# upowai/upow

Hardware: AMD Instinct MI355X
Metric: sha256_pow_hashrate_MH/s (higher is better)
Workload: dtype uint32; 1 GPU; model=upow v2 block header PoW (108 B, single SHA-256, nibble-prefix target), global_batch=4294967296, seq_len=108, parallelism=dp1, nonces_per_rank_step=4294967296, device=gpu, kernel_variant=0

## Files before the change

csrc/bindings.cpp:

```cpp
#include <pybind11/numpy.h>
#include <pybind11/pybind11.h>
#include <pybind11/stl.h>

#include <cstring>
#include <malloc.h>
#include <stdexcept>

#include "native.h"
#include "sha256_common.h"
#include "thread_pool.h"

namespace py = pybind11;
using namespace upow;

namespace upow {
void register_txcodec(py::module_& m);
void register_ledger_writer(py::module_& m);
void register_gov_index(py::module_& m);
void register_stall_probe(py::module_& m);
void register_log_appender(py::module_& m);
void register_http_wire(py::module_& m);
void register_mempool_index(py::module_& m);
void register_jsonspan(py::module_& m);
void register_utxo_host(py::module_& m);
// ... 82 lines not shown
            if (!PyUnicode_Check(o)) throw py::type_error("transaction hex must be str");
            Py_ssize_t sz = 0;
            const char* p = PyUnicode_AsUTF8AndSize(o, &sz);
            if (!p) throw py::error_already_set();
            if (nc[k] < 0 || nc[k] > int64_t(sz)) throw py::value_error("sha256_hex_prefixes: prefix longer than the hex");
            src[size_t(k)] = p;
        }
        std::string out(size_t(n) * 32, '\0');
        {
            py::gil_scoped_release rel;
            HostPool::get().parallel_for(n, threads, [&](int64_t k) {
                host_sha256(reinterpret_cast<const uint8_t*>(src[size_t(k)]), size_t(nc[k]),
                            reinterpret_cast<uint8_t*>(&out[size_t(k) * 32]));
            });
        }
        return py::bytes(out);
    }, py::arg("hexes"), py::arg("idx"), py::arg("nchars"), py::arg("threads") = 1);

    m.def("sha256_batch_gpu", [](py::buffer data, py::buffer offsets) {
        const uint8_t* d; const int64_t* o; int64_t n, nb;
        packed_args(data, offsets, d, o, n, nb);
        std::vector<uint8_t> out;
        {
            py::gil_scoped_release rel;
            out = sha256_batch_gpu(d, nb, o, n);
        }
        return py::bytes(reinterpret_cast<const char*>(out.data()), out.size());
    });

    m.def("pow_check_word", [](py::bytes header, uint32_t tmask, uint32_t tword, uint32_t fs, uint32_t fl,
                               uint32_t v) { return pow_check_word_host(make_job(header, tmask, tword, fs, fl), v); });

    m.def("pow_variant_count", []() { return pow_variant_count(); });
    m.def("pow_job_h0", [](py::bytes header, uint32_t v) { return pow_job_h0_host(make_job(header, 0, 0, 0, 16), v); },
          py::arg("header"), py::arg("v"),
          "digest word H0 for nonce word v, from the precomputed job constants of the GPU kernel (host arithmetic)");

    m.def("pow_job_h0_variant", [](py::bytes header, uint32_t v, int variant) {
              return pow_job_h0_host(make_job(header, 0, 0, 0, 16), v, variant); },
          py::arg("header"), py::arg("v"), py::arg("variant"),
          "pow_job_h0 through the device function of one kernel variant (host arithmetic)");

    m.def("pow_split_consts", [](py::bytes header, uint32_t tmask, uint32_t tword, uint32_t fs, uint32_t fl) {
        const PowSplitConsts c = pow_split_consts(make_job(header, tmask, tword, fs, fl));
        return py::dict(py::arg("ca") = c.ca, py::arg("ce") = c.ce, py::arg("c17") = c.c17, py::arg("c24") = c.c24,
                        py::arg("mid0") = c.mid0, py::arg("range_ok") = c.range_ok,
                        py::arg("range_base") = c.range_base, py::arg("range_width") = c.range_width,
                        py::arg("min_log2") = c.min_log2, py::arg("max_log2") = c.max_log2);
    }, py::arg("header"), py::arg("tmask"), py::arg("tword"), py::arg("frac_shift"), py::arg("frac_limit"),
       "job constants of kernel variant 10 (108-byte header): a11 = ca + v, e11 = ce + v, W17 = c17 + v, "
       "W24 = c24 + v; the range form of the hit predicate, or range_ok False where the job keeps the mask form");

    m.def("pow_range_hit", [](py::bytes header, uint32_t tmask, uint32_t tword, uint32_t fs, uint32_t fl,
                              uint32_t h0) { return pow_range_hit_host(make_job(header, tmask, tword, fs, fl), h0); },
          py::arg("header"), py::arg("tmask"), py::arg("tword"), py::arg("frac_shift"), py::arg("frac_limit"),
          py::arg("h0"), "variant 10's one-compare hit predicate on a digest word H0 (range_ok jobs only)");

    m.def("pow_range_hit_folded", [](py::bytes header, uint32_t tmask, uint32_t tword, uint32_t fs, uint32_t fl,
                                     uint32_t h0) { return pow_range_hit_folded_host(make_job(header, tmask, tword, fs, fl), h0); },
          py::arg("header"), py::arg("tmask"), py::arg("tword"), py::arg("frac_shift"), py::arg("frac_limit"),
          py::arg("h0"), "variant 11's hit compare, range_base folded into round 63's constant (range_ok jobs only)");

    m.def("pow_split_wave", [](py::bytes header, uint32_t vb, uint32_t p, uint32_t u_first, uint32_t iters, int variant) {
        const std::vector<uint32_t> h = pow_split_wave_host(make_job(header, 0, 0, 0, 16), vb, p, u_first, iters, variant);
        py::array_t<uint32_t> out({py::ssize_t(iters), py::ssize_t(64)});
        std::memcpy(out.mutable_data(), h.data(), h.size() * sizeof(uint32_t));
        return out;
    }, py::arg("header"), py::arg("vb"), py::arg("p"), py::arg("u_first"), py::arg("iters"), py::arg("variant") = 0,
       "variant 10's or 11's (0: the default's) wave loop on the host: H0[iteration][lane] for nonce words vb + U + (lane << p), "
       "U = u_first .. u_first + iters - 1, with the kernel's cached lane constants");

    m.def("pow_search_host", [](py::bytes header, uint32_t tmask, uint32_t tword, uint32_t fs, uint32_t fl,
                                uint64_t start, uint64_t count, int threads) {
        PowJobHost j = make_job(header, tmask, tword, fs, fl);
        PowResult r;
        {
            py::gil_scoped_release rel;
            r = pow_search_host(j, start, count, threads);
        }
        return pow_result_tuple(r);
    });

    m.def("pow_search_gpu", [](py::bytes header, uint32_t tmask, uint32_t tword, uint32_t fs, uint32_t fl,
                               uint64_t start, uint64_t count, int grid_blocks, uint32_t chunk_iters, uint32_t cap, int variant) {
        PowJobHost j = make_job(header, tmask, tword, fs, fl);
        PowResult r;
        {
            py::gil_scoped_release rel;
            r = pow_search_gpu(j, start, count, grid_blocks, chunk_iters, cap, variant);
        }
        return pow_result_tuple(r);
    }, py::arg("header"), py::arg("tmask"), py::arg("tword"), py::arg("frac_shift"), py::arg("frac_limit"),
       py::arg("start"), py::arg("count"), py::arg("grid_blocks") = 0, py::arg("chunk_iters") = 0,
       py::arg("cap") = 1 << 16, py::arg("variant") = 0);

    m.def("set_node_device", [](int dev) { set_node_device_native(dev); }, py::arg("device"),
          "pin node-side GPU work (verify, decompress, batched SHA-256) to this device from every thread");
    m.def("pow_kernel_info", [](int variant) {
        PowKernelInfo k = pow_kernel_info(variant);
        return py::dict(py::arg("cus") = k.cus, py::arg("blocks_per_cu") = k.blocks_per_cu,
                        py::arg("resident_blocks") = k.resident_blocks);
    }, py::arg("variant") = 0);
    m.def("p256_verify", [](py::buffer items, bool gpu, int threads) {
        py::buffer_info bi = items.request();
        const int64_t nbytes = bi.size * bi.itemsize;
        if (nbytes % 160) throw std::invalid_argument("items must be n x 160 bytes");
        const int64_t n = nbytes / 160;
        const uint8_t* p = static_cast<const uint8_t*>(bi.ptr);
        std::vector<uint8_t> st;
        {
            py::gil_scoped_release rel;
            st = gpu ? p256_verify_gpu(p, n) : p256_verify_host(p, n, threads);
        }
        return py::bytes(reinterpret_cast<const char*>(st.data()), st.size());
    }, py::arg("items"), py::arg("gpu") = false, py::arg("threads") = 1);

    m.def("p256_decompress", [](py::buffer in, bool gpu) {
        py::buffer_info bi = in.request();
        const int64_t nbytes = bi.size * bi.itemsize;
        if (nbytes % 33) throw std::invalid_argument("input must be n x 33 bytes");
        const int64_t n = nbytes / 33;
        std::vector<uint8_t> out(static_cast<size_t>(n) * 64), ok(static_cast<size_t>(n));
        {
            py::gil_scoped_release rel;
            if (gpu) p256_decompress_gpu(static_cast<const uint8_t*>(bi.ptr), n, out.data(), ok.data());
            else p256_decompress_host(static_cast<const uint8_t*>(bi.ptr), n, out.data(), ok.data());
        }
        return py::make_tuple(py::bytes(reinterpret_cast<const char*>(out.data()), out.size()),
                              py::bytes(reinterpret_cast<const char*>(ok.data()), ok.size()));
    }, py::arg("data"), py::arg("gpu") = false);

    m.def("p256_on_curve", [](py::buffer in, bool gpu, int threads) {
        py::buffer_info bi = in.request();
        const int64_t nbytes = bi.size * bi.itemsize;
        if (nbytes % 64) throw std::invalid_argument("input must be n x 64 bytes (x LE | y LE)");
        const int64_t n = nbytes / 64;
        std::string ok(static_cast<size_t>(n), '\0');
        {
            py::gil_scoped_release rel;
            auto* o = reinterpret_cast<uint8_t*>(&ok[0]);
            if (gpu) p256_on_curve_gpu(static_cast<const uint8_t*>(bi.ptr), n, o);
            else p256_on_curve_host(static_cast<const uint8_t*>(bi.ptr), n, o, threads);
        }
        return py::bytes(ok);
    }, py::arg("data"), py::arg("gpu") = false, py::arg("threads") = 8);

    m.def("p256_pubkey", [](py::bytes d_be) -> py::object {
        std::string d = d_be;
        if (d.size() != 32) throw std::invalid_argument("private key must be 32 bytes big-endian");
        uint8_t out[64];
        if (!p256_pubkey(reinterpret_cast<const uint8_t*>(d.data()), out)) return py::none();
        return py::bytes(reinterpret_cast<const char*>(out), 64);
    });

    m.def("p256_scalar_inv_mont", [](py::bytes s_le) -> py::bytes {
        const std::string s = s_le;
        if (s.size() != 32) throw std::invalid_argument("need 32 bytes little-endian");
        uint64_t in[4], out[4];
        std::memcpy(in, s.data(), 32);
        p256_scalar_inv_mont_host(out, in);
        return py::bytes(reinterpret_cast<const char*>(out), 32);
    });

    m.def("rccl_unique_id", []() { return py::bytes(rccl_unique_id()); });
    m.def("rccl_vote_create", [](py::bytes uid, int world, int rank) {
        const std::string u = uid;
        py::gil_scoped_release rel;
        return rccl_vote_create(u, world, rank);
    });
    m.def("rccl_vote_start", [](int64_t h, int value) { rccl_vote_start(h, value); });
    m.def("rccl_vote_finish", [](int64_t h, double timeout_s) {
        py::gil_scoped_release rel;
        return rccl_vote_finish(h, timeout_s);
    });
    m.def("rccl_vote_stats", [](int64_t h) { return rccl_vote_stats(h); });
    m.def("rccl_vote_destroy", [](int64_t h, bool abort) {
        py::gil_scoped_release rel;
// ... 485 lines not shown
```

csrc/native.h:

```cpp
#pragma once
#include <cstdint>
#include <functional>
#include <string>
#include <vector>

namespace upow {

struct PowJobHost {
    std::vector<uint8_t> header;
    uint32_t tmask = 0, tword = 0, frac_shift = 0, frac_limit = 16;
};

struct PowResult {
    uint64_t searched = 0;
    uint32_t total_hits = 0;
    std::vector<uint32_t> words;
};

struct PowKernelInfo {
    int cus = 0, blocks_per_cu = 0, resident_blocks = 0;
};
PowKernelInfo pow_kernel_info(int variant);
int pow_variant_count();
uint32_t pow_job_h0_host(const PowJobHost& job, uint32_t v);
uint32_t pow_job_h0_host(const PowJobHost& job, uint32_t v, int variant);

struct PowSplitConsts {
    uint32_t ca = 0, ce = 0, c17 = 0, c24 = 0;
    uint32_t mid0 = 0;
    bool range_ok = false;
    uint32_t range_base = 0, range_width = 0;
    int min_log2 = 0, max_log2 = 0;
};
PowSplitConsts pow_split_consts(const PowJobHost& job);
bool pow_range_hit_host(const PowJobHost& job, uint32_t h0);
bool pow_range_hit_folded_host(const PowJobHost& job, uint32_t h0);
std::vector<uint32_t> pow_split_wave_host(const PowJobHost& job, uint32_t vb, uint32_t p, uint32_t u_first,
                                          uint32_t iters, int variant = 0);

bool pow_check_word_host(const PowJobHost& job, uint32_t v);
PowResult pow_search_host(const PowJobHost& job, uint64_t start, uint64_t count, int threads);
PowResult pow_search_gpu(const PowJobHost& job, uint64_t start, uint64_t count, int grid_blocks,
                         uint32_t chunk_iters, uint32_t cap, int variant);

std::vector<uint8_t> sha256_batch_host(const uint8_t* data, const int64_t* offsets, int64_t n, int threads);
std::vector<uint8_t> sha256_batch_gpu(const uint8_t* data, int64_t nbytes, const int64_t* offsets, int64_t n);

std::vector<uint8_t> p256_verify_host(const uint8_t* items, int64_t n, int threads);
uint8_t p256_verify_one_host64(const uint8_t* item);
const void* p256_g_table_host();
void p256_scalar_inv_mont_host(uint64_t out[4], const uint64_t s[4]);
void p256_batch_launch(char variant, const void* items, int64_t n, const void* gtab16, void* scratch, uint8_t* status,
                       int spw, void* stream);
std::string rccl_unique_id();
int64_t rccl_vote_create(const std::string& uid, int world, int rank);
void rccl_vote_start(int64_t h, int value);
int64_t rccl_vote_finish(int64_t h, double timeout_s);
void rccl_vote_destroy(int64_t h, bool abort);
std::vector<double> rccl_vote_stats(int64_t h);
std::vector<uint8_t> p256_g16_entries(int64_t first, int64_t count);
const void* p256_g16_table_device();
std::vector<uint8_t> p256_verify_gpu(const uint8_t* items, int64_t n);
void p256_decompress_host(const uint8_t* in33, int64_t n, uint8_t* out64, uint8_t* ok);
void p256_decompress_gpu(const uint8_t* in33, int64_t n, uint8_t* out64, uint8_t* ok);
void p256_verify_fused_gpu(int64_t n_jobs, int64_t n_out, const std::function<void(uint8_t*, uint8_t*, uint8_t*)>& fill,
                           uint8_t* st, uint8_t* out_ok, std::vector<uint8_t>* items_out);
void p256_on_curve_host(const uint8_t* xy64, int64_t n, uint8_t* ok, int threads);
void p256_on_curve_gpu(const uint8_t* xy64, int64_t n, uint8_t* ok);
void set_node_device_native(int dev);
bool p256_pubkey(const uint8_t d_be[32], uint8_t out_le[64]);
bool p256_sign(const uint8_t d_be[32], const uint8_t digest[32], uint8_t r_le[32], uint8_t s_le[32]);
void p256_pubkey_many_host(const uint8_t* keys_be, int64_t n, uint8_t* out_le, uint8_t* ok, int threads);
void p256_sign_many_host(const uint8_t* keys_be, const uint8_t* digests, int64_t n, uint8_t* rs_le, uint8_t* ok,
                         int threads);
void p256_pubkey_gpu(const uint8_t* keys_be, int64_t n, uint8_t* out_le, uint8_t* ok);
void p256_sign_gpu(const uint8_t* keys_be, const uint8_t* digests, int64_t n, uint8_t* rs_le, uint8_t* ok);
void p256_candidates_host(const uint8_t key_be[32], const uint8_t digest[32], int count, uint8_t* out);
void p256_candidates_gpu(const uint8_t key_be[32], const uint8_t digest[32], int count, uint8_t* out);
struct VanityInfo {
    int keys_per_lane, lanes_per_block, max_ranges;
    int64_t keys_per_launch;
};
VanityInfo p256_vanity_info();
struct VanityHits {
    uint64_t total = 0;
    std::vector<uint64_t> indexes;
};
VanityHits p256_vanity_search(const uint8_t base_be[32], int64_t count, const uint8_t* ranges66, int64_t n_ranges,
                              int64_t max_hits, bool gpu, int threads, int64_t launch_keys, int64_t launch_lanes);
std::vector<uint8_t> p256_vanity_walk(const uint8_t base_be[32], int64_t count, bool gpu, int threads,
                                      int64_t launch_keys, int64_t launch_lanes);
std::vector<uint8_t> p256_probe(const std::string& op, const uint8_t* a, size_t a_bytes, const uint8_t* b, size_t b_bytes,
                                const std::string& mode);
void p256_probe_occ_launch(int op, const uint32_t* a, const uint32_t* b, uint8_t* out, int64_t n, void* stream);

int64_t utxo_create(uint32_t log2_cap);
void utxo_destroy(int64_t h);
uint32_t utxo_capacity(int64_t h);
uint64_t utxo_rehash(int64_t h, uint32_t log2_cap);
uint64_t utxo_insert(int64_t h, const uint8_t* recs, int64_t n, const uint8_t* payload);
std::vector<uint8_t> utxo_probe(int64_t h, const uint8_t* recs, int64_t n);
std::vector<uint8_t> utxo_lookup(int64_t h, const uint8_t* recs, int64_t n, std::vector<uint8_t>& payload_out);
std::vector<uint8_t> utxo_erase(int64_t h, const uint8_t* recs, int64_t n);
struct UtxoSeg { const uint8_t* recs; const uint8_t* pay; int64_t n; };
bool utxo_apply_async(int64_t h, const std::vector<UtxoSeg>& ins, bool with_pay, const uint8_t* del, int64_t n_del,
                      uint32_t prev[3]);
bool utxo_apply_wait(int64_t h, uint32_t out[3]);
std::vector<uint8_t> utxo_dump(int64_t h, std::vector<uint8_t>* payload_out);
void utxo_debug_hashes(const uint8_t* recs, int64_t n, uint32_t log2_cap, uint32_t* home_out, uint64_t* fp_out);
std::vector<uint8_t> utxo_debug_slots(int64_t h);

std::vector<uint8_t> utxo_address_scan(int64_t h, const uint8_t* addr, uint32_t len, uint32_t tag_mask,
                                       uint32_t stake_sel, std::vector<uint8_t>& payload_out, uint64_t* total_out);
struct AddressBatchOut {
    std::vector<uint32_t> qidx;
    std::vector<uint8_t> recs;
    std::vector<uint8_t> payload;
    std::vector<uint64_t> totals;
};
void utxo_address_scan_batch(int64_t h, const uint8_t* addrs, const uint32_t* lens, const uint32_t* tag_masks,
                             const uint32_t* stake_sels, int64_t n, AddressBatchOut& out);

struct OwnerTotalsOut {
    std::vector<uint8_t> recs;
    uint64_t owners = 0, outputs = 0, skipped = 0;
    uint64_t totals[8] = {0, 0, 0, 0, 0, 0, 0, 0};
// ... 68 lines not shown
```

csrc/pow_search.hip:

```cpp
#include <hip/hip_runtime.h>

#include <algorithm>
#include <cstdint>
#include <stdexcept>
#include <string>
#include <utility>

#include "native.h"
#include "streams.h"
#include "sha256_common.h"

namespace upow {

struct PowJobDev {
    uint32_t st[8];
    uint32_t mid[8];
    uint32_t w[16];
    uint32_t tmask;
    uint32_t tword;
    uint32_t frac_shift;
    uint32_t frac_limit;
    uint32_t ca, ce;
    uint32_t hk[3];
    uint32_t kw[64];
    uint32_t c24;
    uint32_t he;
    uint32_t fxg, bxc;
    uint32_t range_ok, range_base, range_width;
};
struct PowFillDev {
    uint32_t k17w;
    uint32_t c33;
    uint32_t k63r;
};
__host__ __device__ __forceinline__ PowFillDev make_pow_fill(const PowJobDev& j) {
    return {kSha256K[17] + j.kw[17], j.kw[33] + j.kw[17], kSha256K[63] + j.range_base};
}

struct PowWordKinds {
    bool vec[64];
    bool has_const[64];
};
constexpr PowWordKinds pow_word_kinds(int layout) {
    PowWordKinds k{};
    for (int i = 0; i < 16; ++i) k.vec[i] = layout == 2 ? i == 10 : (i == 1 || i == 2);
    for (int i = 16; i < 64; ++i) {
        const int src[4] = {i - 16, i - 15, i - 7, i - 2};
        bool v = false, c = false;
        for (int t = 0; t < 4; ++t) {
            if (k.vec[src[t]]) v = true; else c = true;
        }
        k.vec[i] = v;
        k.has_const[i] = v && c;
    }
    return k;
}

#define ROTR(x, n) __builtin_amdgcn_alignbit((x), (x), (n))
#define XOR3(a, b, c) __builtin_amdgcn_bitop3_b32((a), (b), (c), 0x96)
#define BSIG0(x) XOR3(ROTR((x), 2), ROTR((x), 13), ROTR((x), 22))
#define BSIG1(x) XOR3(ROTR((x), 6), ROTR((x), 11), ROTR((x), 25))
#define SSIG0(x) XOR3(ROTR((x), 7), ROTR((x), 18), ((x) >> 3))
#define SSIG1(x) XOR3(ROTR((x), 17), ROTR((x), 19), ((x) >> 10))
#define CH(e, f, g) (((e) & (f)) | (~(e) & (g)))
#define MAJ(a, b, c) __builtin_amdgcn_bitop3_b32((a), (b), (c), 0xE8)

__constant__ uint32_t dK[64] = {
    0x428a2f98u, 0x71374491u, 0xb5c0fbcfu, 0xe9b5dba5u, 0x3956c25bu, 0x59f111f1u, 0x923f82a4u, 0xab1c5ed5u,
    0xd807aa98u, 0x12835b01u, 0x243185beu, 0x550c7dc3u, 0x72be5d74u, 0x80deb1feu, 0x9bdc06a7u, 0xc19bf174u,
    0xe49b69c1u, 0xefbe4786u, 0x0fc19dc6u, 0x240ca1ccu, 0x2de92c6fu, 0x4a7484aau, 0x5cb0a9dcu, 0x76f988dau,
    0x983e5152u, 0xa831c66du, 0xb00327c8u, 0xbf597fc7u, 0xc6e00bf3u, 0xd5a79147u, 0x06ca6351u, 0x14292967u,
    0x27b70a85u, 0x2e1b2138u, 0x4d2c6dfcu, 0x53380d13u, 0x650a7354u, 0x766a0abbu, 0x81c2c92eu, 0x92722c85u,
    0xa2bfe8a1u, 0xa81a664bu, 0xc24b8b70u, 0xc76c51a3u, 0xd192e819u, 0xd6990624u, 0xf40e3585u, 0x106aa070u,
    0x19a4c116u, 0x1e376c08u, 0x2748774cu, 0x34b0bcb5u, 0x391c0cb3u, 0x4ed8aa4au, 0x5b9cca4fu, 0x682e6ff3u,
    0x748f82eeu, 0x78a5636fu, 0x84c87814u, 0x8cc70208u, 0x90befffau, 0xa4506cebu, 0xbef9a3f7u, 0xc67178f2u};

template <int LAYOUT>
__device__ __forceinline__ uint32_t pow_h0(const PowJobDev& job, uint32_t v) {
    constexpr int R0 = LAYOUT == 2 ? 10 : 1;
    uint32_t w[16];
#pragma unroll
    for (int i = 0; i < 16; ++i) w[i] = job.w[i];
    if (LAYOUT == 2) {
        w[10] = v;
    } else {
        w[1] = job.w[1] | ((v & 0xffu) << 8) | ((v >> 8) & 0xffu);
        w[2] = job.w[2] | (((v >> 16) & 0xffu) << 24) | ((v >> 24) << 16);
    }
// ... 752 lines not shown
__global__ __launch_bounds__(256, MIN_WAVES_PER_SIMD) void pow_search_kernel(PowJobDev job, uint32_t v_base, uint32_t iters,
                                                         uint32_t* __restrict__ out_count,
                                                         uint32_t* __restrict__ out_words, uint32_t cap) {
    const uint32_t nthreads = gridDim.x * blockDim.x;
    uint32_t v = v_base + blockIdx.x * blockDim.x + threadIdx.x;
    for (uint32_t it = 0; it < iters; ++it, v += nthreads) {
        const uint32_t h0 = pow_h0<LAYOUT>(job, v);
        const bool hit = ((h0 ^ job.tword) & job.tmask) == 0 && ((h0 >> job.frac_shift) & 0xfu) < job.frac_limit;
        if (__builtin_expect(hit, 0)) {
            const uint32_t slot = atomicAdd(out_count, 1u);
            if (slot < cap) out_words[slot] = v;
        }
    }
}

template <int LAYOUT, int MIN_WAVES_PER_SIMD>
__global__ __launch_bounds__(256, MIN_WAVES_PER_SIMD) void pow_search_pre_kernel(PowJobDev job, uint32_t v_base, uint32_t iters,
                                                             uint32_t* __restrict__ out_count,
                                                             uint32_t* __restrict__ out_words, uint32_t cap) {
    const uint32_t nthreads = gridDim.x * blockDim.x;
    uint32_t v = v_base + blockIdx.x * blockDim.x + threadIdx.x;
    for (uint32_t it = 0; it < iters; ++it, v += nthreads) {
        const uint32_t h0 = pow_h0_pre<LAYOUT>(job, v);
        const bool hit = ((h0 ^ job.tword) & job.tmask) == 0 && ((h0 >> job.frac_shift) & 0xfu) < job.frac_limit;
        if (__builtin_expect(hit, 0)) {
            const uint32_t slot = atomicAdd(out_count, 1u);
            if (slot < cap) out_words[slot] = v;
        }
    }
}

template <int D, bool TWO_PATH, int FILL, int MIN_WAVES_PER_SIMD>
__global__ __launch_bounds__(256, MIN_WAVES_PER_SIMD) void pow_search_sched_kernel(PowJobDev job, uint32_t v_base, uint32_t iters,
                                                               uint32_t* __restrict__ out_count,
                                                               uint32_t* __restrict__ out_words, uint32_t cap) {
    const uint32_t nthreads = gridDim.x * blockDim.x;
    uint32_t v = v_base + blockIdx.x * blockDim.x + threadIdx.x;
    for (uint32_t it = 0; it < iters; ++it, v += nthreads) {
        const uint32_t h0 = pow_h0_sched<2, D, TWO_PATH, FILL>(job, v);
        const bool hit = ((h0 ^ job.tword) & job.tmask) == 0 && ((h0 >> job.frac_shift) & 0xfu) < job.frac_limit;
        if (__builtin_expect(hit, 0)) {
            const uint32_t slot = atomicAdd(out_count, 1u);
            if (slot < cap) out_words[slot] = v;
        }
    }
}

template <bool RANGE>
__global__ __launch_bounds__(256, 7) void pow_search_fill_kernel(PowJobDev job, uint32_t vb, uint32_t p, uint32_t u_begin,
                                                                 uint32_t u_end, uint32_t iters,
                                                                 uint32_t* __restrict__ out_count,
                                                                 uint32_t* __restrict__ out_words, uint32_t cap,
                                                                 PowFillDev fx) {
    const uint32_t wave = blockIdx.x * 4u + __builtin_amdgcn_readfirstlane(threadIdx.x >> 6);
    const uint32_t lane = threadIdx.x & 63u;
    uint32_t u = u_begin + wave * iters;
    if (u >= u_end) return;
    const uint32_t u_stop = u_end - u < iters ? u_end : u + iters;
    PowSplitCacheT<true> cached;
    PowSplitLane lc;
    pow_split_prologue(job, p, vb + u, lane, cached, lc);
    cached.next = __builtin_amdgcn_readfirstlane(cached.next);
    for (; u < u_stop; ++u) {
        const uint32_t sv = vb + u;
        const uint32_t a = pow_a_fill<2>(job, p, sv, lane, cached, lc, fx, RANGE);
        bool hit;
        if (RANGE) {
            hit = a < job.range_width;
        } else {
            const uint32_t h0 = job.mid[0] + a;
            hit = ((h0 ^ job.tword) & job.tmask) == 0 && ((h0 >> job.frac_shift) & 0xfu) < job.frac_limit;
        }
#if defined(__HIP_DEVICE_COMPILE__)
        if (__builtin_expect(__builtin_amdgcn_ballot_w64(hit) != 0, 0)) {
            if (hit) {
                const uint32_t slot = atomicAdd(out_count, 1u);
                if (slot < cap) out_words[slot] = sv + lc.lanep;
            }
        }
#endif
    }
}

template <bool RANGE>
__global__ __launch_bounds__(256, 8) void pow_search_split_kernel(PowJobDev job, uint32_t vb, uint32_t p, uint32_t u_begin,
                                                                  uint32_t u_end, uint32_t iters,
                                                                  uint32_t* __restrict__ out_count,
                                                                  uint32_t* __restrict__ out_words, uint32_t cap) {
    const uint32_t wave = blockIdx.x * 4u + __builtin_amdgcn_readfirstlane(threadIdx.x >> 6);
    const uint32_t lane = threadIdx.x & 63u;
    uint32_t u = u_begin + wave * iters;
    if (u >= u_end) return;
    const uint32_t u_stop = u_end - u < iters ? u_end : u + iters;
    PowSplitCache cached;
    PowSplitLane lc;
    pow_split_prologue(job, p, vb + u, lane, cached, lc);
    for (; u < u_stop; ++u) {
        const uint32_t sv = vb + u;
        const uint32_t a = pow_a_split<2>(job, p, sv, lane, cached, lc);
        bool hit;
        if (RANGE) {
            hit = a + job.range_base < job.range_width;
        } else {
            const uint32_t h0 = job.mid[0] + a;
            hit = ((h0 ^ job.tword) & job.tmask) == 0 && ((h0 >> job.frac_shift) & 0xfu) < job.frac_limit;
        }
        if (__builtin_expect(hit, 0)) {
            const uint32_t slot = atomicAdd(out_count, 1u);
            if (slot < cap) out_words[slot] = sv + lc.lanep;
        }
    }
}

static void hip_check(hipError_t e, const char* what) {
    if (e != hipSuccess) throw std::runtime_error(std::string(what) + ": " + hipGetErrorString(e));
}

constexpr int kPowSplitMinLog2 = 8, kPowSplitMaxLog2 = 26;

PowJobDev make_pow_job(const PowJobHost& hj) {
    PowJobDev j{};
    const uint8_t* hdr = hj.header.data();
    const size_t len = hj.header.size();
    if (len != 108 && len != 138) throw std::invalid_argument("header must be 108 (v2) or 138 (v1) bytes");
    uint32_t st[8];
    std::memcpy(st, kSha256IV, sizeof(st));
    const int full_blocks = len == 108 ? 1 : 2;
    for (int b = 0; b < full_blocks; ++b) host_compress(st, hdr + 64 * b);
    uint8_t tail[64] = {0};
    const size_t rem = len - 64 * full_blocks;
    std::memcpy(tail, hdr + 64 * full_blocks, rem);
    std::memset(tail + rem - 4, 0, 4);
    tail[rem] = 0x80;
    const uint64_t bits = uint64_t(len) * 8;
    for (int i = 0; i < 8; ++i) tail[56 + i] = uint8_t(bits >> (56 - 8 * i));
    for (int i = 0; i < 16; ++i) j.w[i] = load_be32(tail + 4 * i);
    std::memcpy(j.mid, st, sizeof(st));
    uint32_t ws[8];
    std::memcpy(ws, st, sizeof(st));
    host_rounds(ws, j.w, len == 108 ? 10 : 1);
    std::memcpy(j.st, ws, sizeof(ws));
    j.tmask = hj.tmask;
    j.tword = hj.tword;
    j.frac_shift = hj.frac_shift;
    j.frac_limit = hj.frac_limit;
    const int r0 = len == 108 ? 10 : 1;
    const PowWordKinds kinds = pow_word_kinds(len == 108 ? 2 : 1);
    auto ssig0 = [](uint32_t x) { return host_rotr(x, 7) ^ host_rotr(x, 18) ^ (x >> 3); };
    auto ssig1 = [](uint32_t x) { return host_rotr(x, 17) ^ host_rotr(x, 19) ^ (x >> 10); };
    uint32_t wc[64] = {0};
    for (int i = 0; i < 64; ++i) {
        if (i < 16) {
            if (!kinds.vec[i]) wc[i] = j.w[i];
        } else {
            uint32_t sum = 0;
            if (!kinds.vec[i - 16]) sum += wc[i - 16];
            if (!kinds.vec[i - 15]) sum += ssig0(wc[i - 15]);
            if (!kinds.vec[i - 7]) sum += wc[i - 7];
            if (!kinds.vec[i - 2]) sum += ssig1(wc[i - 2]);
            if (!kinds.vec[i]) wc[i] = sum;
            else j.kw[i] = sum;
        }
        if (!kinds.vec[i]) j.kw[i] = kSha256K[i] + wc[i];
    }
    {
        const uint32_t* s = j.st;
        const uint32_t t1 = s[7] + (host_rotr(s[4], 6) ^ host_rotr(s[4], 11) ^ host_rotr(s[4], 25)) +
                            ((s[4] & s[5]) ^ (~s[4] & s[6])) + kSha256K[r0];
        const uint32_t t2 = (host_rotr(s[0], 2) ^ host_rotr(s[0], 13) ^ host_rotr(s[0], 22)) +
                            ((s[0] & s[1]) ^ (s[0] & s[2]) ^ (s[1] & s[2]));
        j.ce = s[3] + t1;
        j.ca = t1 + t2;
        for (int k = 0; k < 3; ++k) {
            const int i = r0 + 1 + k;
            j.hk[k] = s[6 - k] + (kinds.vec[i] ? kSha256K[i] : j.kw[i]);
        }
    }
    j.c24 = j.kw[24] + j.kw[17];
    j.he = j.st[2] + j.hk[0];
    j.fxg = j.st[4] ^ j.st[5];
    j.bxc = j.st[0] ^ j.st[1];
    {
        uint32_t width = 0;
        bool ok = false;
        if (j.frac_limit < 16) {
            const uint32_t above = j.frac_shift + 4 >= 32 ? 0u : ~((1u << (j.frac_shift + 4)) - 1u);
            ok = j.frac_shift <= 28 && j.tmask == above;
            width = j.frac_limit << (j.frac_shift & 31);
        } else if (j.tmask != 0) {
            width = j.tmask & (0u - j.tmask);
            ok = j.tmask == 0u - width;
        }
        ok = ok && width != 0 && (j.tword & ~j.tmask) == 0;
        j.range_ok = ok ? 1 : 0;
        j.range_base = j.mid[0] - j.tword;
        j.range_width = ok ? width : 0;
    }
    return j;
}

PowSplitConsts pow_split_consts(const PowJobHost& hj) {
    if (hj.header.size() != 108) throw std::invalid_argument("the split kernel is for the 108-byte header");
    const PowJobDev j = make_pow_job(hj);
    PowSplitConsts c;
    c.ca = j.ca; c.ce = j.ce; c.c17 = j.kw[17]; c.c24 = j.c24;
    c.mid0 = j.mid[0];
    c.range_ok = j.range_ok != 0;
    c.range_base = j.range_base;
    c.range_width = j.range_width;
    c.min_log2 = kPowSplitMinLog2;
    c.max_log2 = kPowSplitMaxLog2;
    return c;
}

bool pow_range_hit_host(const PowJobHost& hj, uint32_t h0) {
    const PowJobDev j = make_pow_job(hj);
    if (!j.range_ok) throw std::invalid_argument("this job's predicate has no range form");
    const uint32_t a = h0 - j.mid[0];
    return a + j.range_base < j.range_width;
}

template <bool G11>
static std::vector<uint32_t> pow_split_wave_loop(const PowJobDev& job, uint32_t vb, uint32_t p, uint32_t u_first,
                                                 uint32_t iters) {
    PowSplitCacheT<G11> cached[64];
    PowSplitLane lc[64];
    const PowFillDev fx = make_pow_fill(job);
    (void)fx;
    for (uint32_t lane = 0; lane < 64; ++lane) pow_split_prologue(job, p, vb + u_first, lane, cached[lane], lc[lane]);
    std::vector<uint32_t> out(size_t(iters) * 64);
    for (uint32_t it = 0; it < iters; ++it)
        for (uint32_t lane = 0; lane < 64; ++lane) {
            const uint32_t sv = vb + u_first + it;
            if constexpr (G11) out[size_t(it) * 64 + lane] = job.mid[0] + pow_a_fill<2>(job, p, sv, lane, cached[lane], lc[lane], fx, false);
            else out[size_t(it) * 64 + lane] = job.mid[0] + pow_a_split<2>(job, p, sv, lane, cached[lane], lc[lane]);
        }
    return out;
}

std::vector<uint32_t> pow_split_wave_host(const PowJobHost& hj, uint32_t vb, uint32_t p, uint32_t u_first,
                                          uint32_t iters, int variant) {
    if (hj.header.size() != 108) throw std::invalid_argument("the split kernel is for the 108-byte header");
    if (p > uint32_t(kPowSplitMaxLog2)) throw std::invalid_argument("p must be at most 26: the lane index takes six bits");
    if (variant == 0) variant = 11;
    if (variant != 10 && variant != 11) throw std::invalid_argument("the wave loop is variant 10's and variant 11's");
    const PowJobDev job = make_pow_job(hj);
    return variant == 11 ? pow_split_wave_loop<true>(job, vb, p, u_first, iters)
                         : pow_split_wave_loop<false>(job, vb, p, u_first, iters);
}

bool pow_range_hit_folded_host(const PowJobHost& hj, uint32_t h0) {
    const PowJobDev j = make_pow_job(hj);
    if (!j.range_ok) throw std::invalid_argument("this job's predicate has no range form");
    const uint32_t a = h0 - j.mid[0];
    const uint32_t folded = a - kSha256K[63] + make_pow_fill(j).k63r;
    return folded < j.range_width;
}

uint32_t pow_job_h0_host(const PowJobHost& hj, uint32_t v) {
    const PowJobDev job = make_pow_job(hj);
    return hj.header.size() == 108 ? pow_h0_pre<2>(job, v) : pow_h0_pre<1>(job, v);
}

struct PowDeviceBuffers {
    int device = -1;
    uint32_t* d_count = nullptr;
    uint32_t* d_words = nullptr;
    uint32_t cap = 0;
};

static thread_local PowDeviceBuffers g_pow_bufs;

static PowDeviceBuffers& pow_buffers(uint32_t cap) {
    int dev = 0;
    hip_check(hipGetDevice(&dev), "hipGetDevice");
    PowDeviceBuffers& b = g_pow_bufs;
    if (b.device != dev || b.cap < cap) {
        if (b.d_count) { (void)hipFree(b.d_count); (void)hipFree(b.d_words); }
        hip_check(hipMalloc(&b.d_count, sizeof(uint32_t)), "hipMalloc count");
        hip_check(hipMalloc(&b.d_words, sizeof(uint32_t) * cap), "hipMalloc words");
        b.device = dev;
        b.cap = cap;
    }
    return b;
}

constexpr int kPowDefaultVariant = 11;
constexpr int kPowSplitVariant = 10;
constexpr int kPowFillVariant = 11;
constexpr int kPowVariantCount = 12;
static_assert(kPowDefaultVariant == 11, "pow_split_wave_host resolves 0 to the default variant by its number");
static bool pow_is_split(int variant) { return variant == kPowSplitVariant || variant == kPowFillVariant; }

using PowKernelFn = void (*)(PowJobDev, uint32_t, uint32_t, uint32_t*, uint32_t*, uint32_t);

static int pow_resolve_variant(int variant) {
    if (variant < 0 || variant >= kPowVariantCount) throw std::invalid_argument("unknown PoW kernel variant");
    return variant == 0 ? kPowDefaultVariant : variant;
}

static PowKernelFn pow_kernel_fn(bool v2, int variant) {
    variant = pow_resolve_variant(variant);
    if (v2 && pow_is_split(variant)) variant = 9;
    if (!v2) return variant >= 4 ? &pow_search_pre_kernel<1, 7> : &pow_search_kernel<1, 1>;
    switch (variant) {
        case 1: return &pow_search_kernel<2, 8>;
        case 2: return &pow_search_lds_kernel;
        case 4: return &pow_search_pre_kernel<2, 1>;
        case 5: return &pow_search_pre_kernel<2, 8>;
        case 6: return &pow_search_sched_kernel<2, true, 0, 8>;
        case 7: return &pow_search_sched_kernel<2, false, 0, 8>;
        case 8: return &pow_search_sched_kernel<2, false, 1, 8>;
        case 9: return &pow_search_sched_kernel<2, false, 2, 8>;
        default: return &pow_search_kernel<2, 1>;
    }
}

int pow_variant_count() { return kPowVariantCount; }

uint32_t pow_job_h0_host(const PowJobHost& hj, uint32_t v, int variant) {
    if (hj.header.size() != 108) return pow_job_h0_host(hj, v);
    const PowJobDev job = make_pow_job(hj);
    if (variant == 0) variant = kPowDefaultVariant;
    switch (variant) {
        case 6: return pow_h0_sched<2, 2, true, 0>(job, v);
        case 7: return pow_h0_sched<2, 2, false, 0>(job, v);
        case 8: return pow_h0_sched<2, 2, false, 1>(job, v);
        case 9: return pow_h0_sched<2, 2, false, 2>(job, v);
        case 10: return pow_h0_split<false>(job, v);
        case 11: return pow_h0_split<true>(job, v);
        default: return pow_h0_pre<2>(job, v);
    }
}

static int pow_resident_blocks(bool v2, int variant) {
    int dev = 0, cus = 0, per_cu = 0;
    hip_check(hipGetDevice(&dev), "hipGetDevice");
    hip_check(hipDeviceGetAttribute(&cus, hipDeviceAttributeMultiprocessorCount, dev), "attr");
    const int rv = pow_resolve_variant(variant);
    const void* fn = v2 && rv == kPowFillVariant    ? reinterpret_cast<const void*>(&pow_search_fill_kernel<true>)
                     : v2 && rv == kPowSplitVariant ? reinterpret_cast<const void*>(&pow_search_split_kernel<true>)
                                                    : reinterpret_cast<const void*>(pow_kernel_fn(v2, variant));
    hip_check(hipOccupancyMaxActiveBlocksPerMultiprocessor(&per_cu, fn, 256, 0), "occupancy");
    if (per_cu < 1) per_cu = 1;
    if (per_cu > 8) per_cu = 8;
    return cus * per_cu;
}

PowKernelInfo pow_kernel_info(int variant) {
    PowKernelInfo k;
    int dev = 0;
    hip_check(hipGetDevice(&dev), "hipGetDevice");
    hip_check(hipDeviceGetAttribute(&k.cus, hipDeviceAttributeMultiprocessorCount, dev), "attr");
    k.resident_blocks = pow_resident_blocks(true, variant);
    k.blocks_per_cu = k.resident_blocks / (k.cus ? k.cus : 1);
    return k;
}

PowResult pow_search_gpu(const PowJobHost& hj, uint64_t start, uint64_t count, int grid_blocks,
                         uint32_t chunk_iters, uint32_t cap, int variant) {
    PowJobDev job = make_pow_job(hj);
    const bool v2 = hj.header.size() == 108;
    const PowKernelFn kernel = pow_kernel_fn(v2, variant);
    node_device_enter();
    PowDeviceBuffers& buf = pow_buffers(cap);
    hipStream_t st = miner_stream();
    hip_check(hipMemsetAsync(buf.d_count, 0, sizeof(uint32_t), st), "memset");
    const uint32_t block = 256;
    if (grid_blocks <= 0) grid_blocks = pow_resident_blocks(v2, variant);
    const uint64_t per_launch_threads = uint64_t(grid_blocks) * block;
    if (chunk_iters == 0) {
        int lg = node_stream_live().load() ? 23 : 28;
        if (const char* e = std::getenv("UPOW_POW_DISPATCH_LOG2")) lg = std::max(16, std::min(32, std::atoi(e)));
        chunk_iters = uint32_t(std::max<uint64_t>(1, (uint64_t(1) << lg) / per_launch_threads));
    }
    uint64_t done = 0;
    if (v2 && pow_is_split(pow_resolve_variant(variant))) {
        const bool fill = pow_resolve_variant(variant) == kPowFillVariant;
        const auto split = job.range_ok ? &pow_search_split_kernel<true> : &pow_search_split_kernel<false>;
        const auto filled = job.range_ok ? &pow_search_fill_kernel<true> : &pow_search_fill_kernel<false>;
        const PowFillDev fx = make_pow_fill(job);
        const uint64_t waves = uint64_t(grid_blocks) * (block / 64);
        while (count - done >= (uint64_t(1) << (kPowSplitMinLog2 + 6))) {
            int lg = 63 - __builtin_clzll(count - done);
            const uint32_t p = uint32_t(std::min(lg - 6, kPowSplitMaxLog2));
            const uint32_t vb = uint32_t(start + done), n_u = uint32_t(1) << p;
            for (uint32_t u = 0; u < n_u;) {
                const uint32_t left = n_u - u;
                const uint32_t iters = uint32_t(std::min<uint64_t>(chunk_iters, (left + waves - 1) / waves));
                const uint64_t need = (uint64_t(left) + iters - 1) / iters;
                const uint32_t gb = uint32_t(std::min<uint64_t>(uint64_t(grid_blocks), (need + 3) / 4));
                const uint32_t u_end = uint32_t(std::min<uint64_t>(n_u, u + uint64_t(gb) * 4 * iters));
                if (fill)
                    hipLaunchKernelGGL(filled, dim3(gb), dim3(block), 0, st, job, vb, p, u, u_end, iters, buf.d_count,
                                       buf.d_words, cap, fx);
                else
                    hipLaunchKernelGGL(split, dim3(gb), dim3(block), 0, st, job, vb, p, u, u_end, iters, buf.d_count,
                                       buf.d_words, cap);
                hip_check(hipGetLastError(), "pow_search_split_kernel launch");
                u = u_end;
            }
            done += uint64_t(1) << (p + 6);
        }
    }
    while (done < count) {
        const uint64_t left = count - done;
        uint32_t iters = chunk_iters;
        uint32_t gb = grid_blocks;
        if (uint64_t(iters) * per_launch_threads > left) {
            iters = uint32_t(left / per_launch_threads);
            if (iters == 0) {
                iters = 1;
                gb = uint32_t((left + block - 1) / block);
                if (uint64_t(gb) * block > left) {
                    gb = uint32_t(left / block);
                    if (gb == 0) break;
                }
            }
        }
        const uint32_t vb = uint32_t(start + done);
        hipLaunchKernelGGL(kernel, dim3(gb), dim3(block), 0, st, job, vb, iters, buf.d_count, buf.d_words, cap);
        hip_check(hipGetLastError(), "pow_search_kernel launch");
        done += uint64_t(iters) * gb * block;
    }
    uint32_t n = 0;
    hip_check(hipMemcpyAsync(&n, buf.d_count, sizeof(uint32_t), hipMemcpyDeviceToHost, st), "copy count");
    hip_check(hipStreamSynchronize(st), "miner stream sync");
    PowResult r;
    r.searched = done;
    r.total_hits = n;
    const uint32_t stored = n < cap ? n : cap;
    r.words.resize(stored);
    if (stored)
    {
        hip_check(hipMemcpyAsync(r.words.data(), buf.d_words, sizeof(uint32_t) * stored, hipMemcpyDeviceToHost, st),
                  "copy words");
        hip_check(hipStreamSynchronize(st), "miner stream sync");
    }
    if (done < count) {
        for (uint64_t k = done; k < count; ++k) {
            const uint32_t v = uint32_t(start + k);
            if (pow_check_word_host(hj, v)) { r.words.push_back(v); r.total_hits++; }
        }
        r.searched = count;
    }
    return r;
}

}
```

upow_amd/ops/pow.py:

```python
from __future__ import annotations

import hashlib
import os
import time
from dataclasses import dataclass
from typing import List, Optional

from ..models.block import PowTarget
from ..utils import metrics
from .native import gpu_available, lib

NONCE_SPACE = 1 << 32


@dataclass
class PowJob:
    header: bytes
    target: PowTarget
    tmask: int
    tword: int
    frac_shift: int
    frac_limit: int

    @staticmethod
    def create(prefix: bytes, target: PowTarget) -> 'PowJob':
        if len(prefix) not in (104, 134):
            raise ValueError(f'header prefix must be 104 (v2) or 134 (v1) bytes, got {len(prefix)}')
        if target.frac_nibble >= 0 and target.frac_nibble < 8:
            fs, fl = 28 - 4 * target.frac_nibble, target.frac_limit
        else:
            fs, fl = 0, 16
        return PowJob(bytes(prefix) + b'\0\0\0\0', target, target.masks[0], target.words[0], fs, fl)

    @property
    def v2(self) -> bool:
        return len(self.header) == 108

    def word_to_nonce(self, w: int) -> int:
        return int.from_bytes(w.to_bytes(4, 'big'), 'little') if self.v2 else w

    def nonce_to_word(self, n: int) -> int:
        return int.from_bytes(n.to_bytes(4, 'little'), 'big') if self.v2 else n

    def header_with_nonce(self, nonce: int) -> bytes:
        return self.header[:-4] + nonce.to_bytes(4, 'little')

    def exact_check(self, nonce: int) -> bool:
        return self.target.check_hex(hashlib.sha256(self.header_with_nonce(nonce)).hexdigest())

    def native_args(self):
        return (self.header, self.tmask, self.tword, self.frac_shift, self.frac_limit)


@dataclass
class PowSearchResult:
    searched: int
    candidates: int
    nonces: List[int]


def search(job: PowJob, start: int = 0, count: int = NONCE_SPACE, device: Optional[str] = None,
           threads: Optional[int] = None, grid_blocks: int = 0, chunk_iters: int = 0,
           cap: int = 1 << 16, variant: int = 0) -> PowSearchResult:
    L = lib()
    if device is None:
        device = 'gpu' if gpu_available() else 'cpu'
    t0 = time.perf_counter()
    if device == 'gpu':
        searched, hits, words = L.pow_search_gpu(*job.native_args(), start, count, grid_blocks, chunk_iters,
                                                 cap, variant)
    else:
        searched, hits, words = L.pow_search_host(*job.native_args(), start, count,
                                                  threads or max(1, os.cpu_count() or 1))
    dt = time.perf_counter() - t0
    metrics.inc('upow_pow_hashes_total', searched, labels={'device': device}, help='nonces hashed by PoW search')
    if dt > 0:
        metrics.set_gauge('upow_pow_hashrate', searched / dt, labels={'device': device},
                          help='H/s of the last PoW search call')
    nonces = []
    for w in sorted(words):
        n = job.word_to_nonce(w)
        if job.exact_check(n):
            nonces.append(n)
    return PowSearchResult(searched, hits, nonces)
```

Baseline: 39330 MH/s.

## Add dynamic work-claiming persistent kernel variant as default PoW search

```diff
diff --git a/csrc/bindings.cpp b/csrc/bindings.cpp
--- a/csrc/bindings.cpp
+++ b/csrc/bindings.cpp
@@ -188,17 +188,18 @@
     });
 
     m.def("pow_search_gpu", [](py::bytes header, uint32_t tmask, uint32_t tword, uint32_t fs, uint32_t fl,
-                               uint64_t start, uint64_t count, int grid_blocks, uint32_t chunk_iters, uint32_t cap, int variant) {
+                               uint64_t start, uint64_t count, int grid_blocks, uint32_t chunk_iters, uint32_t cap, int variant,
+                               uint32_t claim) {
         PowJobHost j = make_job(header, tmask, tword, fs, fl);
         PowResult r;
         {
             py::gil_scoped_release rel;
-            r = pow_search_gpu(j, start, count, grid_blocks, chunk_iters, cap, variant);
+            r = pow_search_gpu(j, start, count, grid_blocks, chunk_iters, cap, variant, claim);
         }
         return pow_result_tuple(r);
     }, py::arg("header"), py::arg("tmask"), py::arg("tword"), py::arg("frac_shift"), py::arg("frac_limit"),
        py::arg("start"), py::arg("count"), py::arg("grid_blocks") = 0, py::arg("chunk_iters") = 0,
-       py::arg("cap") = 1 << 16, py::arg("variant") = 0);
+       py::arg("cap") = 1 << 16, py::arg("variant") = 0, py::arg("claim") = 0);
 
     m.def("set_node_device", [](int dev) { set_node_device_native(dev); }, py::arg("device"),
           "pin node-side GPU work (verify, decompress, batched SHA-256) to this device from every thread");
diff --git a/csrc/native.h b/csrc/native.h
--- a/csrc/native.h
+++ b/csrc/native.h
@@ -41,7 +41,7 @@
 bool pow_check_word_host(const PowJobHost& job, uint32_t v);
 PowResult pow_search_host(const PowJobHost& job, uint64_t start, uint64_t count, int threads);
 PowResult pow_search_gpu(const PowJobHost& job, uint64_t start, uint64_t count, int grid_blocks,
-                         uint32_t chunk_iters, uint32_t cap, int variant);
+                         uint32_t chunk_iters, uint32_t cap, int variant, uint32_t claim = 0);
 
 std::vector<uint8_t> sha256_batch_host(const uint8_t* data, const int64_t* offsets, int64_t n, int threads);
 std::vector<uint8_t> sha256_batch_gpu(const uint8_t* data, int64_t nbytes, const int64_t* offsets, int64_t n);
diff --git a/csrc/pow_search.hip b/csrc/pow_search.hip
--- a/csrc/pow_search.hip
+++ b/csrc/pow_search.hip
@@ -1,9 +1,11 @@
 #include <hip/hip_runtime.h>
 
 #include <algorithm>
+#include <cstddef>
 #include <cstdint>
 #include <stdexcept>
 #include <string>
+#include <type_traits>
 #include <utility>
 
 #include "native.h"
@@ -922,6 +924,86 @@
     }
 }
 
+struct PowClaimKernArgs {
+    PowJobDev job;
+    uint32_t vb, p, u_begin, u_end, iters;
+    uint32_t *out_count, *out_words;
+    uint32_t cap;
+    PowFillDev fx;
+    uint32_t claim;
+    uint32_t* counter;
+};
+template <bool RANGE>
+__global__ __launch_bounds__(256, 7) void pow_search_claim_kernel(PowJobDev job, uint32_t vb, uint32_t p, uint32_t u_begin,
+                                                                  uint32_t u_end, uint32_t iters,
+                                                                  uint32_t* __restrict__ out_count,
+                                                                  uint32_t* __restrict__ out_words, uint32_t cap,
+                                                                  PowFillDev fx, uint32_t claim, uint32_t* counter) {
+    const uint32_t lane = threadIdx.x & 63u;
+#if defined(__HIP_DEVICE_COMPILE__)
+    for (;;) {
+        auto ka = (__attribute__((address_space(4))) const PowClaimKernArgs*)__builtin_amdgcn_kernarg_segment_ptr();
+        asm volatile("" : "+s"(ka));
+        const uint32_t step = ka->claim, n_u = ka->u_end - ka->u_begin;
+        uint32_t taken = 0;
+        if (lane == 0) taken = __hip_atomic_fetch_add(ka->counter, step, __ATOMIC_RELAXED, __HIP_MEMORY_SCOPE_AGENT);
+        taken = __builtin_amdgcn_readfirstlane(taken);
+        if (taken >= n_u) return;
+        uint32_t u = ka->u_begin + taken;
+        const uint32_t u_stop = n_u - taken < step ? ka->u_end : u + step;
+        PowSplitCacheT<true> cached;
+        PowSplitLane lc;
+        pow_split_prologue(job, p, vb + u, lane, cached, lc);
+        cached.next = __builtin_amdgcn_readfirstlane(cached.next);
+        for (; u < u_stop; ++u) {
+            const uint32_t sv = vb + u;
+            const uint32_t a = pow_a_fill<2>(job, p, sv, lane, cached, lc, fx, RANGE);
+            bool hit;
+            if (RANGE) {
+                hit = a < job.range_width;
+            } else {
+                const uint32_t h0 = job.mid[0] + a;
+                hit = ((h0 ^ job.tword) & job.tmask) == 0 && ((h0 >> job.frac_shift) & 0xfu) < job.frac_limit;
+            }
+            if (__builtin_expect(__builtin_amdgcn_ballot_w64(hit) != 0, 0)) {
+                if (hit) {
+                    const uint32_t slot = atomicAdd(out_count, 1u);
+                    if (slot < cap) out_words[slot] = sv + lc.lanep;
+                }
+            }
+        }
+    }
+#endif
+}
+template <class F>
+struct PowKernargLayout;
+template <class... A>
+struct PowKernargLayout<void (*)(A...)> {
+    static constexpr size_t kCount = sizeof...(A);
+    static constexpr size_t offset(size_t index) {
+        constexpr size_t size[] = {sizeof(A)...}, align[] = {alignof(A)...};
+        size_t at = 0;
+        for (size_t i = 0; i < kCount; ++i) {
+            at = (at + align[i] - 1) / align[i] * align[i];
+            if (i == index) return at;
+            at += size[i];
+        }
+        return at;
+    }
+};
+using PowClaimLayout = PowKernargLayout<decltype(&pow_search_claim_kernel<true>)>;
+static_assert(std::is_same_v<decltype(&pow_search_claim_kernel<true>), decltype(&pow_search_claim_kernel<false>)>);
+static_assert(PowClaimLayout::kCount == 12 && std::is_standard_layout_v<PowClaimKernArgs>);
+static_assert(offsetof(PowClaimKernArgs, job) == PowClaimLayout::offset(0) && offsetof(PowClaimKernArgs, vb) == PowClaimLayout::offset(1) &&
+              offsetof(PowClaimKernArgs, p) == PowClaimLayout::offset(2) && offsetof(PowClaimKernArgs, u_begin) == PowClaimLayout::offset(3) &&
+              offsetof(PowClaimKernArgs, u_end) == PowClaimLayout::offset(4) && offsetof(PowClaimKernArgs, iters) == PowClaimLayout::offset(5) &&
+              offsetof(PowClaimKernArgs, out_count) == PowClaimLayout::offset(6) && offsetof(PowClaimKernArgs, out_words) == PowClaimLayout::offset(7) &&
+              offsetof(PowClaimKernArgs, cap) == PowClaimLayout::offset(8) && offsetof(PowClaimKernArgs, fx) == PowClaimLayout::offset(9) &&
+              offsetof(PowClaimKernArgs, claim) == PowClaimLayout::offset(10) && offsetof(PowClaimKernArgs, counter) == PowClaimLayout::offset(11),
+              "PowClaimKernArgs must mirror pow_search_claim_kernel's parameters");
+static_assert(offsetof(PowClaimKernArgs, u_begin) == 456 && offsetof(PowClaimKernArgs, claim) == 504 &&
+              offsetof(PowClaimKernArgs, counter) == 512, "the offsets in the code object's metadata (.args) at the time of writing");
+
 template <bool RANGE>
 __global__ __launch_bounds__(256, 8) void pow_search_split_kernel(PowJobDev job, uint32_t vb, uint32_t p, uint32_t u_begin,
                                                                   uint32_t u_end, uint32_t iters,
@@ -1082,8 +1164,9 @@
                                           uint32_t iters, int variant) {
     if (hj.header.size() != 108) throw std::invalid_argument("the split kernel is for the 108-byte header");
     if (p > uint32_t(kPowSplitMaxLog2)) throw std::invalid_argument("p must be at most 26: the lane index takes six bits");
-    if (variant == 0) variant = 11;
-    if (variant != 10 && variant != 11) throw std::invalid_argument("the wave loop is variant 10's and variant 11's");
+    if (variant == 0) variant = 12;
+    if (variant == 12) variant = 11;
+    if (variant != 10 && variant != 11) throw std::invalid_argument("the wave loop is variant 10's, 11's and 12's");
     const PowJobDev job = make_pow_job(hj);
     return variant == 11 ? pow_split_wave_loop<true>(job, vb, p, u_first, iters)
                          : pow_split_wave_loop<false>(job, vb, p, u_first, iters);
@@ -1102,6 +1185,7 @@
     return hj.header.size() == 108 ? pow_h0_pre<2>(job, v) : pow_h0_pre<1>(job, v);
 }
 
+constexpr uint32_t kPowClaimCounters = 63;
 struct PowDeviceBuffers {
     int device = -1;
     uint32_t* d_count = nullptr;
@@ -1117,7 +1201,7 @@
     PowDeviceBuffers& b = g_pow_bufs;
     if (b.device != dev || b.cap < cap) {
         if (b.d_count) { (void)hipFree(b.d_count); (void)hipFree(b.d_words); }
-        hip_check(hipMalloc(&b.d_count, sizeof(uint32_t)), "hipMalloc count");
+        hip_check(hipMalloc(&b.d_count, sizeof(uint32_t) * (1 + kPowClaimCounters)), "hipMalloc count");
         hip_check(hipMalloc(&b.d_words, sizeof(uint32_t) * cap), "hipMalloc words");
         b.device = dev;
         b.cap = cap;
@@ -1125,12 +1209,16 @@
     return b;
 }
 
-constexpr int kPowDefaultVariant = 11;
+constexpr int kPowDefaultVariant = 12;
 constexpr int kPowSplitVariant = 10;
 constexpr int kPowFillVariant = 11;
-constexpr int kPowVariantCount = 12;
-static_assert(kPowDefaultVariant == 11, "pow_split_wave_host resolves 0 to the default variant by its number");
-static bool pow_is_split(int variant) { return variant == kPowSplitVariant || variant == kPowFillVariant; }
+constexpr int kPowClaimVariant = 12;
+constexpr int kPowVariantCount = 13;
+constexpr uint32_t kPowClaimDefault = 32;
+static_assert(kPowDefaultVariant == 12, "pow_split_wave_host resolves 0 to the default variant by its number");
+static bool pow_is_split(int variant) {
+    return variant == kPowSplitVariant || variant == kPowFillVariant || variant == kPowClaimVariant;
+}
 
 using PowKernelFn = void (*)(PowJobDev, uint32_t, uint32_t, uint32_t*, uint32_t*, uint32_t);
 
@@ -1168,7 +1256,7 @@
         case 8: return pow_h0_sched<2, 2, false, 1>(job, v);
         case 9: return pow_h0_sched<2, 2, false, 2>(job, v);
         case 10: return pow_h0_split<false>(job, v);
-        case 11: return pow_h0_split<true>(job, v);
+        case 11: case 12: return pow_h0_split<true>(job, v);
         default: return pow_h0_pre<2>(job, v);
     }
 }
@@ -1178,7 +1266,8 @@
     hip_check(hipGetDevice(&dev), "hipGetDevice");
     hip_check(hipDeviceGetAttribute(&cus, hipDeviceAttributeMultiprocessorCount, dev), "attr");
     const int rv = pow_resolve_variant(variant);
-    const void* fn = v2 && rv == kPowFillVariant    ? reinterpret_cast<const void*>(&pow_search_fill_kernel<true>)
+    const void* fn = v2 && rv == kPowClaimVariant   ? reinterpret_cast<const void*>(&pow_search_claim_kernel<true>)
+                     : v2 && rv == kPowFillVariant  ? reinterpret_cast<const void*>(&pow_search_fill_kernel<true>)
                      : v2 && rv == kPowSplitVariant ? reinterpret_cast<const void*>(&pow_search_split_kernel<true>)
                                                     : reinterpret_cast<const void*>(pow_kernel_fn(v2, variant));
     hip_check(hipOccupancyMaxActiveBlocksPerMultiprocessor(&per_cu, fn, 256, 0), "occupancy");
@@ -1198,25 +1287,35 @@
 }
 
 PowResult pow_search_gpu(const PowJobHost& hj, uint64_t start, uint64_t count, int grid_blocks,
-                         uint32_t chunk_iters, uint32_t cap, int variant) {
+                         uint32_t chunk_iters, uint32_t cap, int variant, uint32_t claim) {
     PowJobDev job = make_pow_job(hj);
     const bool v2 = hj.header.size() == 108;
     const PowKernelFn kernel = pow_kernel_fn(v2, variant);
     node_device_enter();
     PowDeviceBuffers& buf = pow_buffers(cap);
     hipStream_t st = miner_stream();
-    hip_check(hipMemsetAsync(buf.d_count, 0, sizeof(uint32_t), st), "memset");
+    const bool claiming = v2 && pow_resolve_variant(variant) == kPowClaimVariant;
+    hip_check(hipMemsetAsync(buf.d_count, 0, sizeof(uint32_t) * (claiming ? 1 + kPowClaimCounters : 1), st), "memset");
     const uint32_t block = 256;
     if (grid_blocks <= 0) grid_blocks = pow_resident_blocks(v2, variant);
     const uint64_t per_launch_threads = uint64_t(grid_blocks) * block;
+    bool whole_pieces = false;
     if (chunk_iters == 0) {
-        int lg = node_stream_live().load() ? 23 : 28;
-        if (const char* e = std::getenv("UPOW_POW_DISPATCH_LOG2")) lg = std::max(16, std::min(32, std::atoi(e)));
+        const bool node = node_stream_live().load();
+        int lg = node ? 23 : 28;
+        const char* e = std::getenv("UPOW_POW_DISPATCH_LOG2");
+        if (e) lg = std::max(16, std::min(32, std::atoi(e)));
+        whole_pieces = claiming && !node && !e;
         chunk_iters = uint32_t(std::max<uint64_t>(1, (uint64_t(1) << lg) / per_launch_threads));
     }
     uint64_t done = 0;
     if (v2 && pow_is_split(pow_resolve_variant(variant))) {
         const bool fill = pow_resolve_variant(variant) == kPowFillVariant;
+        const auto claimed = job.range_ok ? &pow_search_claim_kernel<true> : &pow_search_claim_kernel<false>;
+        if (claiming && claim == 0) {
+            if (const char* e = std::getenv("UPOW_POW_CLAIM")) claim = uint32_t(std::max(0, std::atoi(e)));
+        }
+        uint32_t dispatches = 0;
         const auto split = job.range_ok ? &pow_search_split_kernel<true> : &pow_search_split_kernel<false>;
         const auto filled = job.range_ok ? &pow_search_fill_kernel<true> : &pow_search_fill_kernel<false>;
         const PowFillDev fx = make_pow_fill(job);
@@ -1227,11 +1326,21 @@
             const uint32_t vb = uint32_t(start + done), n_u = uint32_t(1) << p;
             for (uint32_t u = 0; u < n_u;) {
                 const uint32_t left = n_u - u;
-                const uint32_t iters = uint32_t(std::min<uint64_t>(chunk_iters, (left + waves - 1) / waves));
+                const uint32_t iters = uint32_t(std::min<uint64_t>(whole_pieces ? left : chunk_iters, (left + waves - 1) / waves));
                 const uint64_t need = (uint64_t(left) + iters - 1) / iters;
                 const uint32_t gb = uint32_t(std::min<uint64_t>(uint64_t(grid_blocks), (need + 3) / 4));
                 const uint32_t u_end = uint32_t(std::min<uint64_t>(n_u, u + uint64_t(gb) * 4 * iters));
-                if (fill)
+                if (claiming) {
+                    const uint32_t n = u_end - u;
+                    uint32_t c = claim ? claim : std::min(kPowClaimDefault, std::max(1u, iters / 4));
+                    c = uint32_t(std::min<uint64_t>(std::min(c, n), (0xffffffffull - n) / (uint64_t(gb) * 4 + 1)));
+                    c = std::max(c, 1u);
+                    const uint32_t k = dispatches++ % kPowClaimCounters;
+                    if (k == 0 && dispatches > 1)
+                        hip_check(hipMemsetAsync(buf.d_count + 1, 0, sizeof(uint32_t) * kPowClaimCounters, st), "memset claims");
+                    hipLaunchKernelGGL(claimed, dim3(gb), dim3(block), 0, st, job, vb, p, u, u_end, iters, buf.d_count,
+                                       buf.d_words, cap, fx, c, buf.d_count + 1 + k);
+                } else if (fill)
                     hipLaunchKernelGGL(filled, dim3(gb), dim3(block), 0, st, job, vb, p, u, u_end, iters, buf.d_count,
                                        buf.d_words, cap, fx);
                 else
diff --git a/upow_amd/ops/pow.py b/upow_amd/ops/pow.py
--- a/upow_amd/ops/pow.py
+++ b/upow_amd/ops/pow.py
@@ -61,14 +61,14 @@
 
 def search(job: PowJob, start: int = 0, count: int = NONCE_SPACE, device: Optional[str] = None,
            threads: Optional[int] = None, grid_blocks: int = 0, chunk_iters: int = 0,
-           cap: int = 1 << 16, variant: int = 0) -> PowSearchResult:
+           cap: int = 1 << 16, variant: int = 0, claim: int = 0) -> PowSearchResult:
     L = lib()
     if device is None:
         device = 'gpu' if gpu_available() else 'cpu'
     t0 = time.perf_counter()
     if device == 'gpu':
         searched, hits, words = L.pow_search_gpu(*job.native_args(), start, count, grid_blocks, chunk_iters,
-                                                 cap, variant)
+                                                 cap, variant, **({'claim': claim} if claim else {}))
     else:
         searched, hits, words = L.pow_search_host(*job.native_args(), start, count,
                                                   threads or max(1, os.cpu_count() or 1))
```

Measured after the change: 42570 MH/s, median of 6. 8.3% higher.
